# jatinagwal/kyverno

Measured on AMD Instinct MI355X. Metric: resource×rule evals/sec (background scan, PSS+best-practices) at 1/2/4/8 GPUs, higher is better.
Workload: dtype u32

## Files before the change

### __graft_entry__.py

```python
import os
import subprocess
import sys

ROOT = os.path.dirname(os.path.abspath(__file__))
if ROOT not in sys.path:
    sys.path.insert(0, ROOT)


def build():
    from kyverno_amd import build as B
    B.build()
    subprocess.run(["make", "-C", os.path.join(ROOT, "oracle"), "-j8"], check=True)
    import kyverno_amd
    from kyverno_amd import _lib
    _lib.lib()
    try:
        import concurrent.futures
        cache = os.path.join(ROOT, "kyverno_amd", "jitcache")
        jobs = [(wl, a) for wl in ("c3", "tests-c3", "c5", "c4", "c2") for a in (False, True)]
        try:
            sys.path.insert(0, os.path.join(ROOT, "tests"))
            import table_edge_cases
            jobs += [("tests-edges:%d" % i, False) for i in range(len(table_edge_cases.compiled_rulesets()))]
            import meta_keys_cases
            jobs += [("tests-metakeys%s:%d" % (off, i), a) for i in range(len(meta_keys_cases.compiled_rulesets()))
                     for off in ("", "-off") for a in (False, True)]
        except Exception as e:
            print("build: test rulesets not compiled ahead of time: %s" % e, file=sys.stderr)
        ctx = __import__("multiprocessing").get_context("spawn")
        with concurrent.futures.ProcessPoolExecutor(max_workers=min(len(jobs), os.cpu_count() or 1, 16), mp_context=ctx) as ex:
            list(ex.map(_aot_compile, jobs))
        t_start = {}
        ents = [f for f in os.listdir(cache) if f.endswith(".co")]
        for kind in ("walk", "acct"):
            newest = max((f for f in ents if f.startswith(kind + "-")), key=lambda f: os.path.getmtime(os.path.join(cache, f)))
            t_start[kind] = newest.split("-")[1]
        for f in os.listdir(cache):
            parts = f.split("-")
            if f.endswith(".co") and (len(parts) != 3 or t_start.get(parts[0]) != parts[1]):
                os.remove(os.path.join(cache, f))
    except Exception as e:
        print("build: ahead-of-time walk-kernel compile skipped: %s" % e, file=sys.stderr)
    try:
        _cache_bench_corpus()
    except Exception as e:
        print("build: bench corpus not prebuilt: %s" % e, file=sys.stderr)


def _cache_bench_corpus(total=10_000_000, need_free=14 << 30):
    import shutil
    import bench
    from kyverno_amd import synth
    if synth.corpus_is_cached(bench.CORPUS_CACHE, total, kind="mixed", seed=bench.SEED):
        return
    os.makedirs(bench.CORPUS_CACHE, exist_ok=True)
    free = shutil.disk_usage(bench.CORPUS_CACHE).free
    if free < need_free:
        raise RuntimeError("%.0f GB free under %s, %.0f GB wanted" % (free / 2**30, bench.CORPUS_CACHE, need_free / 2**30))
    synth.write_corpus_cache(bench.CORPUS_CACHE, total, kind="mixed", seed=bench.SEED)


def _aot_compile(job):
    if ROOT not in sys.path:
        sys.path.insert(0, ROOT)
    sys.path.insert(0, os.path.join(ROOT, "tests"))
    import bench
    import cases
    from kyverno_amd import engine as E
    wl, acct = job
    if wl.startswith("tests-edges:"):
        import table_edge_cases
        pols = table_edge_cases.compiled_rulesets()[int(wl.split(":")[1])]
    elif wl.startswith("tests-metakeys"):
        import meta_keys_cases
        pols = meta_keys_cases.compiled_rulesets()[int(wl.split(":")[1])]
        if wl.startswith("tests-metakeys-off:"):
            os.environ["KYV_META_KEYS"] = "0"
            try:
                return E.Ruleset(pols).jit_compile(accounting=acct)
            finally:
                del os.environ["KYV_META_KEYS"]
    else:
        pols = cases.best_practices() + cases.chart_restricted() if wl == "tests-c3" else bench.load_policies(wl)
    return E.Ruleset(pols).jit_compile(accounting=acct)


def smoke():
    sys.path.insert(0, os.path.join(ROOT, "tests"))
    import cases
    import parity_util as PU
    from kyverno_amd import synth

    docs, nsl = synth.mixed(300, seed=5, edge=True)
    pols = cases.best_practices()[:4] + cases.chart_restricted()[:6] + cases.quirk_policies()[-2:]
    st, res = PU.compare(pols, docs, nsl, backend="gpu")
    if st["nbad"]:
        raise AssertionError("GPU verdicts differ from the oracle: %r" % (st["bad"][:5],))
    if st["compared"] == 0:
        raise AssertionError("smoke compared no pairs")
    print("smoke ok: %d pairs, %d compared bit-exact vs oracle, kernel %.3f ms" % (st["pairs"], st["compared"],
                                                                                   res.kernel_ms))


if __name__ == "__main__":
    build() if (len(sys.argv) > 1 and sys.argv[1] == "build") else smoke()
```

### kyverno_amd/csrc/jit.cpp

```cpp
#include <dlfcn.h>
#include <sys/stat.h>
#include <unistd.h>
#include <hip/hip_runtime.h>
#include <hip/hiprtc.h>

#include <algorithm>
#include <chrono>
#include <cstdio>
#include <cstdlib>
#include <functional>
#include <map>
#include <mutex>
#include <utime.h>
#include <set>
#include <sstream>
#include <unordered_map>
#include <stdexcept>
#include <string>
#include <vector>

#include "kyv_host.h"

namespace kyv {

int pattern_depth(const Ruleset& rs, uint32_t pn, int guard);

bool jit_meta_keys_on() {
  const char* e = getenv("KYV_META_KEYS");
  return !e || atoi(e) != 0;
}

namespace {

struct Gen {
  const Ruleset& rs;
  std::ostringstream out;
  std::vector<uint8_t> emitted;
  std::vector<uint32_t> emitted_log;
  bool ok = true;
  const bool use_len = !getenv("KYV_JIT_LEN") || atoi(getenv("KYV_JIT_LEN")) != 0;
  const size_t batch_max = getenv("KYV_JIT_BATCH") ? (size_t)std::max(1, atoi(getenv("KYV_JIT_BATCH"))) : 1;
  const bool leaf_fast = !getenv("KYV_JIT_LEAF_FAST") || atoi(getenv("KYV_JIT_LEAF_FAST")) != 0;
  const bool meta_keys;
  static constexpr uint32_t MK_COL = 0x80000000u;
  struct WildSrc { int pc = -1; bool two = false; uint32_t cs = 0; };
  std::vector<int> slot_meta;
  std::vector<WildSrc> wild_src;
  WildSrc cur_src[MAX_SLOTS];
  int class_of(uint32_t pn) const {
    const PNode& P = rs.pnodes[pn];
    if (!meta_keys || !(P.flags & PF_META) || node_mbase[pn] == NONE || meta_pos[pn] < 0) return -1;
    const size_t s = (size_t)node_mbase[pn] + P.meta;
    return s < rs.meta_class_of.size() ? rs.meta_class_of[s] : -1;
  }

  std::vector<int> slot;
  std::vector<int> slot_alen;
  std::vector<int> slot_elen;
  std::vector<std::vector<uint32_t>> scope_of;
  std::vector<uint8_t> scoped;
  std::vector<uint32_t> node_mbase;
  std::vector<int8_t> meta_pos;

  explicit Gen(const Ruleset& r, int meta_keys_mode = -1)
      : rs(r), meta_keys(meta_keys_mode < 0 ? jit_meta_keys_on() : meta_keys_mode != 0), emitted(r.pnodes.size(), 0), slot_meta(r.pnodes.size(), -1), wild_src(r.pentries.size()),
        slot(r.pentries.size(), -1), slot_alen(r.pnodes.size(), -1),
        slot_elen(r.pentries.size(), -1), scope_of(r.pnodes.size()), scoped(r.pnodes.size(), 0),
        node_mbase(r.pnodes.size(), NONE), meta_pos(r.pnodes.size(), -1) {}

  void mark_paths(uint32_t pn, uint32_t mbase, uint32_t k0, uint32_t k1, uint32_t k2, uint32_t k3, int depth) {
    if (pn == NONE || pn >= rs.pnodes.size() || depth > 4) return;
    const PNode& P = rs.pnodes[pn];
    if (P.kind != P_MAP) return;
    node_mbase[pn] = mbase;
    const uint32_t S = SID_FIRST_FREE + K_SPEC, T = SID_FIRST_FREE + K_TEMPLATE, J = SID_FIRST_FREE + K_JOBTEMPLATE;
    if (depth == 0) meta_pos[pn] = 0;
    else if (depth == 2 && k0 == S && k1 == T) meta_pos[pn] = 1;
    else if (depth == 4 && k0 == S && k1 == J && k2 == S && k3 == T) meta_pos[pn] = 2;
    for (uint32_t e = 0; e < P.n; e++) {
      const PEntry& E = rs.pentries[P.first + e];
      if ((E.flags & EF_WILD) || E.child == NONE || E.handler == H_STAR || E.handler == H_NEGATION ||
          E.handler == H_EXISTENCE || E.handler == H_EXIST_BADPAT)
// ... 438 lines not shown
          out << "  if (" << c << " != NONE) return mkerr(EC_NONE, 0, " << ET << ");\n";
          break;
        case H_EXISTENCE: {
          uint32_t npat = rs.pool[E.child];
          out << "  if (" << c << " != NONE) {\n"
              << "    uint32_t cnt, eb, aa = NONE;\n";
          if (slot_elen[P.first + e] >= 0)
            out << "    if (" << t << " == N_ARR && (uint32_t)(pc[" << slot_elen[P.first + e] << "] >> 32) != NONE) {\n"
                << "      cnt = (uint32_t)pc[" << slot_elen[P.first + e] << "]; eb = (uint32_t)(pc[" << slot_elen[P.first + e]
                << "] >> 32);\n"
                << "    } else\n";
          out << "    { const Node a = gnode(w.R + " << c << ");\n"
              << "      if (node_type(a) != N_ARR) return mkerr(EC_NONE, 0, " << ET << ");\n"
              << "      cnt = a.b; eb = a.c; aa = a.a; }\n";
          for (uint32_t j = 0; j < npat; j++) {
            out << "    { bool hit = false;\n"
                << "      for (uint32_t i = 0; i < cnt; i++) {\n"
                << "        const uint32_t er = eb == NONE ? NONE : eb + i;\n"
                << "        " << preload(rs.pool[E.child + 1 + j], "pe", "er") << "\n"
                << "        uint32_t et = T_UNK, ea = 0u, ei = NONE;\n"
                << (rs.pe_self[P.first + e] != NONE ? "        ei = jdec(jself(w, " + u(rs.pe_self[P.first + e]) + ", er), &et, &ea);\n"
                                                      : std::string())
                << "        if (ei == NONE) { ei = aa + i; et = T_UNK; }\n"
                << "        Ret r = p" << rs.pool[E.child + 1 + j] << "(w, ei, et, ea, er, pe);\n"
                << "        if (w.ost) return r;\n"
                << "        if (!r.err) { hit = true; break; }\n"
                << "      }\n"
                << "      if (!hit) return mkerr(EC_NONE, 0, " << ET << "); }\n";
          }
          out << "  }\n";
          break;
        }
        default:
          out << "  {\n";
          call("");
          out << "  }\n";
      }
    }
    out << "  return ok_ret();\n";
  }
};

struct CondGen {
  const Ruleset& rs;
  std::ostringstream defs;
  std::ostringstream out;
  bool ok = true;
  uint32_t uid = 0;
  uint32_t nslots = 1;
  bool lds_used = false;
  uint32_t cur_etpos = NONE;
  std::unordered_map<uint64_t, std::string> progs;

  explicit CondGen(const Ruleset& r) : rs(r) {}
  static std::string u(uint32_t x) { return std::to_string(x) + "u"; }
  std::string fresh(const char* p) { return std::string(p) + std::to_string(uid++); }

  uint32_t tchild(uint32_t t, uint32_t key) const {
    if (t == NONE) return NONE;
    for (auto& kv : rs.trie[t].kids) if (kv.first == key) return kv.second;
    return NONE;
  }
  uint32_t tstar(uint32_t t) const { return t == NONE ? NONE : rs.trie[t].star; }
  uint32_t tcol(uint32_t t) const { return t == NONE ? NONE : rs.trie[t].col; }
  uint32_t tlen(uint32_t t) const { return t == NONE || rs.trie[t].star == NONE ? NONE : rs.trie[t].lencol; }

  struct V {
    std::string i, t, a, row;
    uint32_t tpos;
    bool key;
  };
  V decl(const std::string& i, const std::string& t, const std::string& a, const std::string& row, uint32_t tpos,
         bool key) {
    V x{fresh("vi"), fresh("vt"), fresh("va"), fresh("vr"), tpos, key};
    out << "  uint32_t " << x.i << " = " << i << ", " << x.t << " = " << t << ", " << x.a << " = " << a << ", " << x.row
        << " = " << row << ";\n";
    return x;
  }
  V field(const V& x, uint32_t key) {
    if (x.key) return decl("NONE", "T_UNK", "0u", "NONE", NONE, false);
    const uint32_t ct = tchild(x.tpos, key), col = tcol(ct);
    V y{fresh("vi"), fresh("vt"), fresh("va"), fresh("vr"), col == NONE ? NONE : ct, false};
    out << "  uint32_t " << y.i << ", " << y.t << ", " << y.a << ";\n"
        << "  jc_field(v, R, " << x.i << ", " << x.row << ", " << (col == NONE ? "NONE" : u(col)) << ", " << u(key) << ", &"
        << y.i << ", &" << y.t << ", &" << y.a << ");\n"
        << "  const uint32_t " << y.row << " = " << (col == NONE ? std::string("NONE") : x.row) << ";\n";
    return y;
  }
  bool unroll = false;
  V open_elems(const V& x, const std::string& notarr_then, const char* on_arr = "") {
    const std::string cnt = fresh("cn"), aa = fresh("aa"), eb = fresh("eb"), j = fresh("j");
    const uint32_t st = tstar(x.tpos);
    out << "  { uint32_t " << cnt << " = 0u, " << aa << " = 0u, " << eb << " = NONE;\n"
        << "  if (" << (x.key ? "false" : "jc_arr(v, R, " + x.i + ", " + x.t + ", " + x.a + ", " + x.row + ", " +
                                              (tlen(x.tpos) == NONE ? std::string("NONE") : u(tlen(x.tpos))) + ", &" + cnt +
                                              ", &" + aa + ", &" + eb + ")")
        << ") {\n" << on_arr << (unroll ? "  KYV_JC_UNROLL\n" : "")
        << "  for (uint32_t " << j << " = 0; " << j << " < " << cnt << "; " << j << "++) {\n";
    V e{fresh("vi"), fresh("vt"), fresh("va"), fresh("vr"), st, false};
    out << "  uint32_t " << e.i << ", " << e.t << ", " << e.a << ", " << e.row << ";\n"
        << "  jc_elem(v, R, " << aa << ", " << (st == NONE ? std::string("NONE") : eb) << ", " << j << ", "
        << (tcol(st) == NONE ? std::string("NONE") : u(tcol(st))) << ", &" << e.i << ", &" << e.t << ", &" << e.a << ", &"
        << e.row << ");\n";
    pending_else.push_back(notarr_then);
    return e;
  }
  std::vector<std::string> pending_else;
  void close_loop() {
    out << "  }\n  }";
    std::string e = pending_else.back();
    pending_else.pop_back();
    if (!e.empty()) out << " else {\n" << e << "  }";
    out << "\n  }\n";
  }

  const uint32_t* P = nullptr;
  uint32_t PN = 0, PEND = 0;
  bool streaming = false;
  std::string sacc;
  void jend(const V& x, bool list, bool proj) {
    if (!list) {
      out << "  *cur = " << (x.key ? "(" + x.i + " | JMES_KEYBIT)" : x.i) << ";\n";
      return;
    }
    if (streaming) {
      std::string sx;
      if (x.key) sx = "(gtk(R + " + x.i + ") >> 4)";
      else sx = "jc_sprint(R, " + x.i + ", " + x.t + ", " + x.a + ")";
      const std::string body = "{ const uint32_t es = " + sx + ";\n    if (++*ln > JCAP) return JS_FB;\n    " + sacc + " }";
      if (x.key) out << "  " << body << "\n";
      else if (proj) out << "  if (" << x.i << " != NONE) " << body << "\n";
      else out << "  " << body << "\n";
      return;
    }
    const std::string e = x.key ? "jc_keyent(R, " + x.i + ")" : "jc_ent(" + x.i + ", " + x.t + ", " + x.a + ")";
    if (x.key) out << "  if (!jc_push(L, ln, " << e << ")) return JS_FB;\n";
    else if (proj) out << "  if (" << x.i << " != NONE) { if (!jc_push(L, ln, " << e << ")) return JS_FB; }\n";
    else out << "  if (!jc_push(L, ln, " << x.i << " == NONE ? NONE : " << e << ")) return JS_FB;\n";
  }
  void jgen(uint32_t pos, const V& x, bool list, bool proj, int guard) {
    if (!ok || guard > 64) { ok = false; return; }
    if (pos >= PEND) { jend(x, list, proj); return; }
    const uint32_t op = P[pos];
    switch (op) {
      case JO_FIELD: {
        out << "  {\n";
        V y = field(x, P[pos + 1]);
        jgen(pos + 2, y, list, proj, guard + 1);
        out << "  }\n";
        return;
      }
      case JO_MULTI: {
        if (list) { ok = false; return; }
        const uint32_t m = P[pos + 1];
        out << "  if (" << x.i << " == NONE) {\n";
        jgen(pos + 2 + m, x, false, proj, guard + 1);
        out << "  } else {\n  *lst = true;\n";
        for (uint32_t o = 0; o < m; o++) {
          out << "  {\n";
          V y = field(x, P[pos + 2 + o]);
          jgen(pos + 2 + m, y, true, proj, guard + 1);
          out << "  }\n";
        }
        out << "  }\n";
        return;
      }
      case JO_FLAT: {
        if (!list) {
          std::ostringstream save;
          save.swap(out);
          V nul{"NONE", "T_UNK", "0u", "NONE", NONE, false};
          jgen(pos + 1, nul, false, false, guard + 1);
          std::string notarr = out.str();
          out.swap(save);
          V e = open_elems(x, notarr, "  *lst = true;\n");
          jgen(pos + 1, e, true, true, guard + 1);
          close_loop();
          return;
        }
        out << "  if (" << (proj && !x.key ? x.i + " != NONE" : std::string("true")) << ") {\n";
        std::ostringstream save;
        save.swap(out);
        V pass{x.i, x.t, x.a, "NONE", NONE, x.key};
        jgen(pos + 1, pass, true, true, guard + 1);
        std::string notarr = out.str();
        out.swap(save);
        V e = open_elems(x, notarr);
        jgen(pos + 1, e, true, true, guard + 1);
        close_loop();
        out << "  }\n";
        return;
      }
      case JO_KEYS: {
        if (list) { ok = false; return; }
// ... 326 lines not shown
         << "(const View& v, const Node* R, uint32_t r, uint32_t ei, uint32_t et, uint32_t ea, uint32_t erow, uint32_t* L) {\n"
         << "  (void)ei; (void)et; (void)ea; (void)erow;\n"
         << b << "}\n";
    progs[key] = name;
    return name;
  }

  const ForeachEntry* FE = nullptr;
  void elem_body(const V& e) {
    out << "  do {\n";
    if (FE->scope == 2) out << "  if (jc_type(R, " << e.i << ", " << e.t << ") != N_MAP) return ST_ERROR | ST_MARK_SCOPE;\n";
    out << "  bool err = false;\n";
    const std::string args = "(v, R, r, " + e.i + ", " + e.t + ", " + e.a + ", " + e.row + ", L)";
    if (FE->pre != NONE) {
      const std::string f = prog_fn(FE->pre, e.tpos);
      out << "  { const int c = " << f << args << ";\n"
          << "    if (c == CR_FB) return ST_FALLBACK;\n    if (c == CR_PANIC) return ST_PANIC;\n"
          << "    if (c == CR_FALSE) break;\n    err = c == CP_ERROR; }\n";
    }
    const std::string f = prog_fn(FE->deny, e.tpos);
    out << "  if (!err) { const int c = " << f << args << ";\n"
        << "    if (c == CR_FB) return ST_FALLBACK;\n    if (c == CR_PANIC) return ST_PANIC;\n"
        << "    if (c == CR_TRUE) return ST_FAIL;\n    if (c != CP_ERROR) { count++; break; } }\n"
        << "  pend = true;\n  } while (0);\n";
  }
  void fend(const V& x, bool list, bool proj) {
    if (x.key) { ok = false; return; }
    if (list) {
      if (proj) {
        out << "  if (" << x.i << " != NONE) {\n  pend = false;\n";
        elem_body(x);
        out << "  }\n";
      } else {
        out << "  pend = false;\n  if (" << x.i << " != NONE) {\n";
        elem_body(x);
        out << "  }\n";
      }
      return;
    }
    std::ostringstream save;
    save.swap(out);
    out << "  pend = false;\n  if (" << (x.i == "NONE" ? std::string("false") : x.i + " != NONE && jc_type(R, " + x.i + ", " + x.t + ") != N_NULL")
        << ") {\n";
    elem_body(x);
    out << "  }\n";
    const std::string single = out.str();
    out.swap(save);
    V e = open_elems(x, single);
    out << "  pend = false;\n  if (" << e.i << " != NONE) {\n";
    elem_body(e);
    out << "  }\n";
    close_loop();
  }
  void fgen(uint32_t pos, const V& x, bool list, bool proj, int guard) {
    if (!ok || guard > 64) { ok = false; return; }
    if (pos >= PEND) { fend(x, list, proj); return; }
    const uint32_t op = P[pos];
    switch (op) {
      case JO_FIELD: {
        out << "  {\n";
        V y = field(x, P[pos + 1]);
        fgen(pos + 2, y, list, proj, guard + 1);
        out << "  }\n";
        return;
      }
      case JO_MULTI: {
        if (list) { ok = false; return; }
        const uint32_t m = P[pos + 1];
        out << "  if (" << x.i << " == NONE) {\n";
        fgen(pos + 2 + m, x, false, proj, guard + 1);
        out << "  } else {\n";
        for (uint32_t o = 0; o < m; o++) {
          out << "  {\n";
          V y = field(x, P[pos + 2 + o]);
          fgen(pos + 2 + m, y, true, proj, guard + 1);
          out << "  }\n";
        }
        out << "  }\n";
        return;
      }
      case JO_FLAT: {
        std::ostringstream save;
        save.swap(out);
        if (!list) {
          V nul{"NONE", "T_UNK", "0u", "NONE", NONE, false};
          fgen(pos + 1, nul, false, false, guard + 1);
        } else {
          V pass{x.i, x.t, x.a, "NONE", NONE, x.key};
          fgen(pos + 1, pass, true, true, guard + 1);
        }
        const std::string notarr = out.str();
        out.swap(save);
        if (list) out << "  if (" << (proj ? x.i + " != NONE" : std::string("true")) << ") {\n";
        V e = open_elems(x, notarr);
        fgen(pos + 1, e, true, true, guard + 1);
        close_loop();
        if (list) out << "  }\n";
        return;
      }
      default: ok = false; return;
    }
  }
  void foreach_entry(const ForeachEntry& fe) {
    FE = &fe;
    out << "  { uint32_t count = 0u; bool pend = false; bool skip = false; (void)skip;\n";
    const CondOperand& o = fe.list;
    const uint32_t* p = o.kind == OK_JMES ? rs.pool.data() + o.a : nullptr;
    const bool chain = o.kind == OK_PATH || (p && (p[0] & JF_PURE));
// ... 104 lines not shown
  const uint32_t nany = p.nany == NONE ? 0u : p.nany;
  for (uint32_t i = 0; i < nany; i++)
    if (heavy_jmes(rs, rs.conds[p.any0 + i].key) || heavy_jmes(rs, rs.conds[p.any0 + i].value)) return true;
  for (uint32_t i = 0; i < p.nall; i++)
    if (heavy_jmes(rs, rs.conds[p.all0 + i].key) || heavy_jmes(rs, rs.conds[p.all0 + i].value)) return true;
  return false;
}

std::string self_dir() {
  Dl_info info;
  if (dladdr((void*)&self_dir, &info) && info.dli_fname) {
    std::string p = info.dli_fname;
    size_t s = p.rfind('/');
    return s == std::string::npos ? std::string(".") : p.substr(0, s);
  }
  return ".";
}

}

constexpr uint32_t kFusedGW = 8;
bool jit_rule_fused(const Ruleset& rs, uint32_t k) {
  static const bool on = !getenv("KYV_FUSED") || atoi(getenv("KYV_FUSED")) != 0;
  if (!on || k >= rs.rules.size() || rs.rules.size() > 32u * kFusedGW) return false;
  const RuleDesc& rd = rs.rules[k];
  return (rd.kind == RK_PATTERN || rd.kind == RK_ANYPATTERN) && (rd.flags & RD_GATE_EXACT);
}

bool jit_shape_eligible(const Ruleset& rs, uint32_t k) {
  static const bool on = !getenv("KYV_SHAPES") || atoi(getenv("KYV_SHAPES")) != 0;
  if (!on || k >= rs.rules.size()) return false;
  const RuleDesc& rd = rs.rules[k];
  return rd.kind == RK_PATTERN && rd.pre == NONE && !(rd.flags & RD_GATE_EXACT) && !jit_rule_fused(rs, k);
}

static std::string meta_signature(const Ruleset& rs, const RuleDesc& rd) {
  std::string o;
  if (!rd.uses_meta) return o;
  auto pool = [&](uint32_t at, uint32_t n) {
    for (uint32_t i = 0; i < 2 * n && at + i < rs.pool.size(); i++) o += std::to_string(rs.pool[at + i]) + ",";
  };
  for (uint32_t i = 0; i < rd.nmeta && rd.meta_sites + i < rs.metas.size(); i++) {
    const MetaSite& m = rs.metas[rd.meta_sites + i];
    o += "[" + std::to_string(m.has_labels) + "," + std::to_string(m.has_ann) + "," + std::to_string(m.nwild_l) + ":";
    pool(m.wild_l, m.nwild_l);
    o += std::to_string(m.nwild_a) + ":";
    pool(m.wild_a, m.nwild_a);
    o += std::to_string(m.slot_l) + "," + std::to_string(m.slot_a) + "]";
  }
  return o;
}

std::string jit_source(const Ruleset& rs, std::vector<uint8_t>* jit_rules, std::vector<uint8_t>* jit_cond,
                       std::vector<uint16_t>* jit_shape, int meta_keys) {
  Gen g(rs, meta_keys);
  jit_rules->assign(rs.rules.size(), 0);
  if (jit_shape) jit_shape->assign(rs.rules.size(), 0);
  if (jit_cond) jit_cond->assign(rs.rules.size(), 0);
  const size_t cap = getenv("KYV_JIT_MAX_RULES") ? (size_t)atol(getenv("KYV_JIT_MAX_RULES")) : 1024;
  CondGen cg(rs);
  std::vector<uint32_t> crules;
  const bool cond_on = !getenv("KYV_JIT_COND") || atoi(getenv("KYV_JIT_COND")) != 0;
  for (size_t k = 0; k < rs.rules.size() && cond_on && crules.size() < cap; k++) {
    const RuleDesc& rd = rs.rules[k];
    if (rd.kind != RK_DENY && rd.kind != RK_FOREACH) continue;
    if (rd.kind == RK_DENY && !prog_has_jmes(rs, rd.pre) && !prog_has_jmes(rs, rd.root)) continue;
    const std::string mark = cg.defs.str();
    const auto progs = cg.progs;
    cg.ok = true;
    cg.rule_fn((uint32_t)k);
    if (!cg.ok) {
      cg.defs.str("");
      cg.defs.clear();
      cg.defs << mark;
      cg.progs = progs;
      continue;
    }
    crules.push_back((uint32_t)k);
  }
  std::vector<std::pair<uint32_t, std::vector<uint32_t>>> rule_roots;
  std::ostringstream body;
  std::unordered_map<std::string, uint32_t> shapes;
  std::unordered_map<uint32_t, uint32_t> rep_of;
  auto canon = [](const std::string& t) {
    std::unordered_map<std::string, size_t> ids;
    std::string o;
    o.reserve(t.size());
    for (size_t i = 0; i < t.size();) {
      if (t[i] == 'p' && (i == 0 || !(isalnum((unsigned char)t[i - 1]) || t[i - 1] == '_')) && i + 1 < t.size() &&
          isdigit((unsigned char)t[i + 1])) {
        size_t j = i + 1;
        while (j < t.size() && isdigit((unsigned char)t[j])) j++;
        if (j < t.size() && t[j] == '(') {
          auto it = ids.emplace(t.substr(i, j - i), ids.size()).first;
          o += "p#" + std::to_string(it->second);
          i = j;
          continue;
        }
      }
      o += t[i++];
    }
    return o;
  };
  size_t nshapes = 0;
  const bool only_cond = getenv("KYV_JIT_ONLY_COND") && atoi(getenv("KYV_JIT_ONLY_COND")) != 0;
  for (size_t k = 0; k < rs.rules.size() && !only_cond; k++) {
    const RuleDesc& rd = rs.rules[k];
    if (rd.kind != RK_PATTERN && rd.kind != RK_ANYPATTERN) continue;
    std::vector<uint32_t> rr;
    if (rd.kind == RK_PATTERN) rr.push_back(rd.root);
    else for (uint32_t a = 0; a < rd.nalts; a++) rr.push_back(rs.pool[rd.root + a]);
    bool ok = true;
    for (uint32_t r : rr) if (pattern_depth(rs, r, 0) > MAX_DEPTH) ok = false;
// ... 644 lines not shown
```

### kyverno_amd/csrc/kyv_engine.hip

```cpp
#define KYV_SEL_INLINE 1
#include <hip/hip_runtime.h>

#include <algorithm>
#include <array>
#include <map>
#include <chrono>
#include <cmath>
#include <functional>
#include <cstdlib>
#include <mutex>
#include <set>
#include <cstdio>
#include <cstring>
#include <stdexcept>
#include <string>
#include <thread>
#include <vector>

#include "kyv_acct.h"
#include "kyv_host.h"
#define KYV_NO_KERNELS 1
#include "kyv_kernels.h"

namespace kyv {
// ... 765 lines not shown
    }
    out[(size_t)s * words + w] = bits;
  }
}

int pattern_depth(const Ruleset& rs, uint32_t pn, int guard) {
  if (pn == NONE || guard > MAX_DEPTH) return MAX_DEPTH + 1;
  const PNode& P = rs.pnodes[pn];
  int d = 0;
  switch (P.kind) {
    case P_MAP:
      for (uint32_t e = 0; e < P.n; e++) {
        const PEntry& E = rs.pentries[P.first + e];
        if (E.handler == H_STAR || E.handler == H_NEGATION || E.child == NONE) continue;
        if (E.handler == H_EXISTENCE || E.handler == H_EXIST_BADPAT) {
          uint32_t npat = rs.pool[E.child];
          for (uint32_t j = 0; j < npat; j++) d = std::max(d, 1 + pattern_depth(rs, rs.pool[E.child + 1 + j], guard + 2));
        } else {
          d = std::max(d, pattern_depth(rs, E.child, guard + 1));
        }
      }
      return 1 + d;
    case P_ARR_MAPS: return 1 + pattern_depth(rs, P.first, guard + 1);
    case P_ARR_POS:
      for (uint32_t i = 0; i < P.n; i++) d = std::max(d, pattern_depth(rs, rs.pool[P.first + i], guard + 1));
      return 1 + d;
    default: return 0;
  }
}

static int ruleset_depth(const Ruleset& rs) {
  int d = 1;
  for (auto& rd : rs.rules) {
    if (rd.kind == RK_PATTERN) d = std::max(d, pattern_depth(rs, rd.root, 0));
    else if (rd.kind == RK_ANYPATTERN)
      for (uint32_t a = 0; a < rd.nalts; a++) d = std::max(d, pattern_depth(rs, rs.pool[rd.root + a], 0));
  }
  return std::min(d, (int)MAX_DEPTH);
}


static std::mutex g_jit_mu;
static void mrs_clear_shapes(Ruleset& rs) {
  std::fill(rs.jit_shape.begin(), rs.jit_shape.end(), (uint16_t)0);
  rs.jit_nshapes = 0;
}
static bool ensure_jit(Ruleset& rs, DevRuleset* dr) {
  if (dr->jloaded) return true;
  std::lock_guard<std::mutex> lk(g_jit_mu);
  if (!rs.jit_tried) {
    rs.jit_tried = true;
    try {
      rs.jit_meta_keys = jit_meta_keys_on() && !rs.meta_classes.empty();
      std::string src = jit_source(rs, &rs.jit_rules, &rs.jit_cond, &rs.jit_shape, rs.jit_meta_keys ? 1 : 0);
      rs.jit_nshapes = 0;
      for (auto x : rs.jit_shape) rs.jit_nshapes = std::max<uint32_t>(rs.jit_nshapes, x);
      bool any = false;
      for (auto x : rs.jit_rules) any |= x != 0;
      for (auto x : rs.jit_cond) any |= x != 0;
      if (any) rs.jit_code = jit_compile(src, &rs.jit_compile_s);
    } catch (std::exception& e) {
      rs.jit_error = e.what();
      rs.jit_code.clear();
      fprintf(stderr, "[kyvgpu] runtime-compiled walk kernel unavailable, using the interpreted one: %s\n", e.what());
    }
  }
  if (rs.jit_code.empty()) return false;
  HIP_OK(hipModuleLoadData(&dr->jmod, rs.jit_code.data()));
  uint32_t ng = 0;
  for (auto x : rs.jit_rules) ng = std::max<uint32_t>(ng, x);
  dr->jfns.resize(ng);
  dr->ffns.assign(ng, nullptr);
  for (uint32_t g = 0; g < ng; g++) {
    HIP_OK(hipModuleGetFunction(&dr->jfns[g], dr->jmod, ("kyv_jit_walk_" + std::to_string(g)).c_str()));
    if (hipModuleGetFunction(&dr->ffns[g], dr->jmod, ("kyv_jit_fused_" + std::to_string(g)).c_str()) != hipSuccess)
      dr->ffns[g] = nullptr;
    dr->fparts.resize(ng);
    for (int p = 1; dr->ffns[g]; p++) {
      hipFunction_t f = nullptr;
      if (hipModuleGetFunction(&f, dr->jmod, ("kyv_jit_fused_" + std::to_string(g) + "p" + std::to_string(p)).c_str()) != hipSuccess)
        break;
      dr->fparts[g].push_back(f);
    }
    dr->fmfns.resize(ng, nullptr);
    if (hipModuleGetFunction(&dr->fmfns[g], dr->jmod, ("kyv_jit_fusedm_" + std::to_string(g)).c_str()) != hipSuccess)
      dr->fmfns[g] = nullptr;
  }
  (void)hipGetLastError();
  dr->jshapes = nullptr;
  if (rs.jit_nshapes && hipModuleGetFunction(&dr->jshapes, dr->jmod, "kyv_jit_shapes") != hipSuccess) {
    dr->jshapes = nullptr;
    mrs_clear_shapes(rs);
  }
  (void)hipGetLastError();
  dr->jconds.assign(rs.rules.size(), nullptr);
  dr->jc_group.assign(rs.rules.size(), -1);
  dr->jcg.clear();
  dr->jcg_members.clear();
  {
    std::vector<uint32_t> crules;
    for (size_t k = 0; k < rs.jit_cond.size(); k++) if (rs.jit_cond[k] == 1) crules.push_back((uint32_t)k);
    for (auto& grp : jit_cond_groups(rs, crules)) {
      hipFunction_t f = nullptr;
      if (hipModuleGetFunction(&f, dr->jmod, ("kyv_jit_condg_" + std::to_string(grp[0])).c_str()) != hipSuccess) continue;
      for (uint32_t k : grp) dr->jc_group[k] = (int32_t)dr->jcg.size();
      dr->jcg.push_back(f);
      dr->jcg_members.push_back(grp);
    }
    (void)hipGetLastError();
  }
  for (size_t k = 0; k < rs.jit_cond.size(); k++)
    if (rs.jit_cond[k] == 1 && dr->jc_group[k] < 0)
      HIP_OK(hipModuleGetFunction(&dr->jconds[k], dr->jmod, ("kyv_jit_cond_" + std::to_string(k)).c_str()));
  dr->jloaded = true;
  return true;
}

static bool ensure_jit_acct(Ruleset& rs, DevRuleset* dr) {
  if (dr->aloaded) return true;
  if (!ensure_jit(rs, dr)) return false;
  std::lock_guard<std::mutex> lk(g_jit_mu);
  if (rs.jit_code_acct.empty()) {
    std::vector<uint8_t> jr, jc;
    rs.jit_code_acct = jit_compile(jit_source(rs, &jr, &jc, nullptr, rs.jit_meta_keys ? 1 : 0), nullptr, true);
  }
  HIP_OK(hipModuleLoadData(&dr->amod, rs.jit_code_acct.data()));
  dr->afns.resize(dr->jfns.size());
  dr->affns.assign(dr->jfns.size(), nullptr);
  for (size_t g = 0; g < dr->jfns.size(); g++) {
    HIP_OK(hipModuleGetFunction(&dr->afns[g], dr->amod, ("kyv_jit_walk_" + std::to_string(g)).c_str()));
    if (dr->ffns[g]) HIP_OK(hipModuleGetFunction(&dr->affns[g], dr->amod, ("kyv_jit_fused_" + std::to_string(g)).c_str()));
    dr->afparts.resize(dr->jfns.size());
    dr->afparts[g].assign(g < dr->fparts.size() ? dr->fparts[g].size() : 0, nullptr);
    for (size_t p = 0; p < dr->afparts[g].size(); p++)
      HIP_OK(hipModuleGetFunction(&dr->afparts[g][p], dr->amod,
                                  ("kyv_jit_fused_" + std::to_string(g) + "p" + std::to_string(p + 1)).c_str()));
    dr->afmfns.resize(dr->jfns.size(), nullptr);
    if (g < dr->fmfns.size() && dr->fmfns[g])
      HIP_OK(hipModuleGetFunction(&dr->afmfns[g], dr->amod, ("kyv_jit_fusedm_" + std::to_string(g)).c_str()));
  }
  dr->aconds.assign(dr->jconds.size(), nullptr);
  for (size_t k = 0; k < dr->jconds.size(); k++)
    if (dr->jconds[k]) HIP_OK(hipModuleGetFunction(&dr->aconds[k], dr->amod, ("kyv_jit_cond_" + std::to_string(k)).c_str()));
  dr->ajshapes = nullptr;
  if (dr->jshapes) HIP_OK(hipModuleGetFunction(&dr->ajshapes, dr->amod, "kyv_jit_shapes"));
  dr->ajcg.assign(dr->jcg.size(), nullptr);
  for (size_t g = 0; g < dr->jcg.size(); g++)
    HIP_OK(hipModuleGetFunction(&dr->ajcg[g], dr->amod, ("kyv_jit_condg_" + std::to_string(dr->jcg_members[g][0])).c_str()));
  hipDeviceptr_t p = nullptr;
  size_t bytes = 0;
  HIP_OK(hipModuleGetGlobal(&p, &bytes, dr->amod, "kyv_acct_bytes"));
  dr->acnt = (unsigned long long*)p;
  dr->aloaded = true;
  return true;
}

static size_t rule_slice_bytes(const RuleDesc& rd) {
  const size_t alts = rd.kind == RK_PATTERN ? 1 : rd.kind == RK_ANYPATTERN ? std::min<uint32_t>(rd.nalts, MAX_ALTS) : 0;
  return sizeof(uint2) + 2 * alts * sizeof(FailRec) + 1;
}

static size_t slice_budget() {
  if (const char* e = getenv("KYV_SLICE_MB")) return (size_t)std::max(1, atoi(e)) << 20;
  size_t fr = 0, tot = 0;
  if (hipMemGetInfo(&fr, &tot) != hipSuccess || fr == 0) fr = (size_t)64 << 30;
  return std::min<size_t>(fr / 2, (size_t)128 << 30);
}

static void build_mrec(const Ruleset& rs, uint32_t q, const std::vector<uint32_t>& gidx, bool masks_on, bool on, MRec& R) {
  memset(&R, 0, sizeof R);
  const RuleDesc& rd = rs.rules[q];
  R.k = q;
  R.kind = rd.kind;
  R.flags = rd.flags;
  bool fast = on && rd.match.mode != MM_NONE && rd.exc == NONE && rd.match.nfilters + rd.exclude.nfilters <= MREC_F;
  bool uses = false;
  auto pat = [&](uint32_t sid) -> uint32_t {
// ... 1799 lines not shown
```

### kyverno_amd/csrc/kyv_host.h

```cpp
#pragma once
#include <cstdint>
#include <functional>
#include <memory>
#include <string>
#include <unordered_map>
#include <vector>

#include "kyv_layout.h"
#include "pjson.h"

namespace kyv {

template <class T>
struct NoInitAlloc : std::allocator<T> {
  template <class U> struct rebind { using other = NoInitAlloc<U>; };
  NoInitAlloc() = default;
  template <class U> NoInitAlloc(const NoInitAlloc<U>&) noexcept {}
  template <class U> void construct(U* p) noexcept { ::new ((void*)p) U; }
  template <class U, class... A> void construct(U* p, A&&... a) { ::new ((void*)p) U(std::forward<A>(a)...); }
};
template <class T> using bulk_vector = std::vector<T, NoInitAlloc<T>>;

struct Dict {
  std::vector<std::string> strs;
// ... 50 lines not shown
  std::vector<uint16_t> next;
  std::vector<uint8_t> accept;
  bool end_anchor = false;
};
bool rx_compile(const std::string& re, RxDfa* out, std::string* why);
int rx_match(const RxDfa& d, const uint8_t* s, size_t n);

struct Ruleset {
  Dict dict;
  std::vector<RuleDesc> rules;
  std::vector<RuleMeta> meta;
  std::vector<PolicyMeta> policies;
  std::vector<Filter> filters;
  std::vector<KindDesc> kinds;
  std::vector<SelDesc> sels;
  std::vector<SelReq> reqs;
  std::vector<PNode> pnodes;
  std::vector<PEntry> pentries;
  std::vector<Leaf> leaves;
  std::vector<Atom> atoms;
  std::vector<MetaSite> metas;
  std::vector<PssDesc> pss;
  std::vector<uint32_t> pool;
  std::vector<Node> cnodes;
  std::vector<Cond> conds;
  std::vector<CondProg> cprogs;
  std::vector<CondText> cond_text;
  std::vector<std::string> templates;
  std::unordered_map<std::string, uint32_t> template_ids;
  struct TrieNode {
    uint32_t col = NONE;
    uint32_t rowspace = 0;
    uint32_t star = NONE;
    uint32_t lencol = NONE;
    std::vector<std::pair<uint32_t, uint32_t>> kids;
  };
  std::vector<TrieNode> trie;
  std::vector<uint32_t> gpats;
  std::vector<std::vector<uint32_t>> gsets;
  std::vector<uint32_t> cond_set;
  std::vector<std::string> rx_src;
  std::vector<RxDfa> rxs;
  bool uses_upper = false;
  uint32_t ncols = 0, nrowspaces = 1;
  std::vector<uint32_t> col_rowspace;
  std::vector<uint32_t> pn_self;
  std::vector<uint32_t> pe_self;
  std::vector<uint32_t> pn_len;
  std::vector<uint32_t> pe_len;
  std::vector<uint32_t> fact_spaces;
  std::vector<MetaClass> meta_classes;
  std::vector<int8_t> meta_class_of;
  bool jit_meta_keys = false;
  bool jit_tried = false;
  std::vector<uint8_t> jit_rules;
  std::vector<uint8_t> jit_cond;
  std::vector<uint16_t> jit_shape;
  uint32_t jit_nshapes = 0;
  std::vector<char> jit_code;
  std::vector<char> jit_code_acct;
  std::string jit_error;
  double jit_compile_s = 0;
  std::vector<void*> dev;
  ~Ruleset();
};

struct TypedDecoder {
  enum Target { POD = 0, DEPLOYMENT = 1, CRONJOB = 2 };
  explicit TypedDecoder(const std::function<uint32_t(const std::string&)>& find_sid);
  enum Outcome { DEC_OK = 0, DEC_ERR = 1, DEC_FOLD = 2 };
  int decode(const Node* R, const std::vector<std::string>& strs, int target) const;
  std::unordered_map<uint32_t, uint32_t> name_of_sid;
};

struct Batch {
  const Ruleset* rs = nullptr;
  Dict dict;
  bulk_vector<Node> nodes;
  bulk_vector<ResHeader> hdr;
  bulk_vector<HotHdr> hot;
  std::vector<FloatAux> faux;
  std::vector<uint32_t> str_off, str_len, str_flags;
  std::vector<uint32_t> str_upper, str_rx;
  std::vector<int64_t> str_dur, str_qty;
  std::vector<double> str_f64;
  std::vector<uint8_t> heap;
  std::vector<uint32_t> nsl_off, nsl_kv;
  std::vector<std::string> nsl_names;
  std::vector<uint32_t> order;
  std::vector<uint32_t> inv;
  std::vector<uint64_t> shape_key;
  std::shared_ptr<const std::vector<uint32_t>> inv_shared;
  std::vector<uint32_t> gate;
  uint32_t gate_words = 0, nclass = 0;
  bulk_vector<uint64_t> colv;
  std::vector<uint32_t> col_off, rs_rows;
  std::vector<WaveFacts> facts;
  std::vector<void*> dev;
  ~Batch();
};

struct FailPath {
  uint32_t res, rule, alt;
  uint32_t tmpl;
  uint16_t idx[MAX_IDX];
  uint32_t key[2];
};

struct SlicePlan { uint32_t k0 = 0, k1 = 0, fused = 0, chunk = 0, cond = 0; };
struct EvalPlan {
  uint32_t gmask_patterns = 0, cond_sets = 0, gmask_words = 0, unmasked = 0;
  uint32_t onemask = 0;
  uint32_t tail_used[5] = {0, 0, 0, 0, 0};
  uint32_t tail_cand[5] = {0, 0, 0, 0, 0};
  uint32_t fast = 0, fasteval = 0, generic = 0;
};
void plan_ruleset(const Ruleset& rs, EvalPlan* p);

struct Results {
  uint32_t nres = 0, nrules = 0;
  EvalPlan plan;
  std::vector<SlicePlan> slices;
  std::vector<uint8_t> status;
  std::vector<uint32_t> pss_fails;
  std::vector<FailRec> fails;
  int64_t counts[NSTATUS] = {0};
  std::vector<int64_t> rule_counts;
  double kernel_ms = 0, h2d_ms = 0, d2h_ms = 0;
  double gmask_ms = 0;
  double meta_keys_ms = 0;
  double phase_ms[5] = {0, 0, 0, 0, 0};
  uint64_t alg_bytes = 0;
  uint64_t alg_bytes_phase[5] = {0, 0, 0, 0, 0};
  uint64_t alg_bytes_class[3] = {0, 0, 0};
  int jit_used = 0;
};

Ruleset* compile_ruleset(const char* json, size_t len, std::string* err, const char* exceptions = nullptr,
                         size_t ex_len = 0, bool background = false);
Batch* build_batch(const Ruleset* rs, const char* json, size_t len, const char* nsl_json, size_t nsl_len, int threads,
                   std::string* err);
void derive_strings(Batch& b, size_t from, int threads);
void build_path_trie(Ruleset& rs);
void assign_wave_facts(Ruleset& rs);
void assign_meta_classes(Ruleset& rs);
bool jit_meta_keys_on();
std::vector<MetaKeyRow> meta_key_rows_host(const Ruleset& rs, const Batch& b);
std::vector<MetaKeyRow> meta_key_rows_device(const Batch& b, int device);
size_t meta_key_plane_bytes(const Batch& b);
uint32_t wave_maps_mask();
void assign_glob_masks(Ruleset& rs);
void assign_cond_sets(Ruleset& rs);
std::string jit_source(const Ruleset& rs, std::vector<uint8_t>* jit_rules, std::vector<uint8_t>* jit_cond = nullptr,
                       std::vector<uint16_t>* jit_shape = nullptr, int meta_keys = -1);
bool jit_shape_eligible(const Ruleset& rs, uint32_t k);
constexpr uint32_t JIT_MAX_SHAPES = 64;
std::vector<char> jit_compile(const std::string& src, double* seconds, bool acct = false);
bool jit_rule_fused(const Ruleset& rs, uint32_t k);
std::vector<std::vector<uint32_t>> jit_cond_groups(const Ruleset& rs, const std::vector<uint32_t>& crules);
struct KindGate {
  bool any = false;
  std::vector<uint32_t> kinds;
};
KindGate rule_gate(const Ruleset& rs, const RuleDesc& rd);
enum JitMode { JIT_AUTO = 0, JIT_OFF = 1, JIT_ON = 2 };
constexpr size_t JIT_AUTO_MIN_RESOURCES = 65536;
void resolve_path_columns(Batch& b, int threads);
constexpr uint32_t SHAPE_KEY_BITS = 3, SHAPE_KEY_MAX_NODES = 64 / SHAPE_KEY_BITS;
std::vector<uint32_t> shape_key_nodes(const Ruleset& rs);
std::string format_path(const Ruleset& rs, const Batch& b, uint32_t tmpl, const uint16_t* idx, const uint32_t* key);

}
```

### kyverno_amd/csrc/kyv_jcond.h

```cpp
#pragma once
#include "kyv_wave.h"
#include "kyv_cond.h"
#include "kyv_pss.h"

namespace kyv {

constexpr uint32_t JCAP = 16;

__device__ __forceinline__ uint64_t jc_col(const View& v, uint32_t col, uint32_t row) {
  if (row == NONE) return COL_NONE;
  KYV_ACCT_ADDK(2u, 0, 8);
  const uint32_t off = sld32(v.col_off + col);
  return gcol(v.colv, off, row);
}
__device__ __forceinline__ kyv_u32x4 jc_meta(const View& v, uint32_t cls, uint32_t row) {
  if (row == NONE) return kyv_u32x4{0u, NONE, NONE, NONE};
  KYV_ACCT_ADD(0, 16);
  return *(const KYV_AS_GLOBAL kyv_u32x4*)(v.meta_rows + ((size_t)cls * v.nres + row));
}
__device__ __forceinline__ uint32_t jc_dec(uint64_t x, uint32_t* t, uint32_t* a) {
  const uint32_t lo = (uint32_t)x;
  *a = (uint32_t)(x >> 32);
  if (lo == NONE) { *t = T_UNK; *a = 0; return NONE; }
  *t = lo >> COL_TYPE_SHIFT;
  return lo & COL_INDEX_MASK;
}
__device__ __forceinline__ uint32_t jc_type(const Node* R, uint32_t i, uint32_t t) {
  if (i == NONE) return N_NULL;
  return t != T_UNK ? t : (gtk(R + i) & 0xFu);
}
__device__ __forceinline__ void jc_field(const View& v, const Node* R, uint32_t i, uint32_t row, uint32_t col, uint32_t key,
                                         uint32_t* oi, uint32_t* ot, uint32_t* oa) {
  *ot = T_UNK;
  *oa = 0;
  if (col != NONE && row != NONE) {
    uint32_t x = jc_dec(jc_col(v, col, row), ot, oa);
    if (x != NONE && *ot == N_NULL) { x = NONE; *ot = T_UNK; *oa = 0; }
    *oi = x;
    return;
  }
  if (i == NONE) { *oi = NONE; return; }
  const Node m = gnode(R + i);
  if (node_type(m) != N_MAP) { *oi = NONE; return; }
  const uint32_t x = wmap_find(R, m.a, m.b, key);
  if (x == NONE) { *oi = NONE; return; }
  const Node n = gnode(R + x);
  if (node_type(n) == N_NULL) { *oi = NONE; return; }
  *oi = x;
  *ot = node_type(n);
  *oa = n.a;
}
__device__ __forceinline__ bool jc_arr(const View& v, const Node* R, uint32_t i, uint32_t t, uint32_t a, uint32_t row,
                                       uint32_t lencol, uint32_t* cnt, uint32_t* aa, uint32_t* eb) {
  if (i == NONE) return false;
  if (t != T_UNK && t != N_ARR) return false;
  if (t == N_ARR && lencol != NONE && row != NONE) {
    const uint64_t x = jc_col(v, lencol, row);
    if ((uint32_t)x != NONE) { *cnt = (uint32_t)x; *eb = (uint32_t)(x >> 32); *aa = a; return true; }
  }
  const Node n = gnode(R + i);
  if (node_type(n) != N_ARR) return false;
  *cnt = n.b;
  *aa = n.a;
  *eb = n.c;
  return true;
}
__device__ __forceinline__ void jc_elem(const View& v, const Node* R, uint32_t aa, uint32_t eb, uint32_t j, uint32_t self,
                                        uint32_t* oi, uint32_t* ot, uint32_t* oa, uint32_t* orow) {
  *oi = aa + j;
  *ot = T_UNK;
  *oa = 0;
  *orow = eb == NONE ? NONE : eb + j;
  if (self != NONE && *orow != NONE) {
    uint32_t t, a;
    if (jc_dec(jc_col(v, self, *orow), &t, &a) != NONE) { *ot = t; *oa = a; }
  }
  if (jc_type(R, *oi, *ot) == N_NULL) { *oi = NONE; *ot = T_UNK; *oa = 0; }
}
__device__ __forceinline__ uint32_t jc_ent(uint32_t i, uint32_t t, uint32_t a) {
  return (t == N_STR && a < JMES_SIDBIT) ? (a | JMES_SIDBIT) : i;
}
__device__ __forceinline__ uint32_t jc_keyent(const Node* R, uint32_t idx) {
  const uint32_t k = gtk(R + idx) >> 4;
  return k < JMES_SIDBIT ? (k | JMES_SIDBIT) : (idx | JMES_KEYBIT);
}
__device__ __forceinline__ bool jc_push(uint32_t* L, uint32_t* n, uint32_t e) {
  if (*n >= JCAP) return false;
  L[(size_t)*n << 6] = e;
  (*n)++;
  return true;
}
__device__ __forceinline__ bool jc_false1(const Node* R, uint32_t cur) {
  if (cur == NONE) return true;
  if (cur & JMES_KEYBIT) return node_key(gnode(R + (cur & ~JMES_KEYBIT))) == SID_EMPTY;
  const Node n = gnode(R + cur);
  switch (node_type(n)) {
    case N_NULL: case N_FALSE: return true;
    case N_STR: return n.a == SID_EMPTY;
    case N_ARR: case N_MAP: return n.b == 0;
    default: return false;
  }
}
__device__ __forceinline__ uint32_t jc_sprint(const Node* R, uint32_t i, uint32_t t, uint32_t a) {
// ... 41 lines not shown
```

Baseline: 146.8 billion.

## Collapse chained field lookups into a single preloaded column read in JIT conditions

The condition JIT generator now defers consecutive field accesses along a path whose final trie node has a precomputed column. It emits one column lookup for the whole chain, and falls back to walking the tree node by node only when no row is available. The aim is to replace several dependent global-memory node reads per path with a single column read. It adds an environment switch, a code-generation path that keeps lazy chain state, and extra ahead-of-time test compile jobs. Correctness depends on the column encoding matching the result of the full chain walk.

Measured after the change: 152.0 billion, median of 6. +3.6%, better.

```diff
diff --git a/__graft_entry__.py b/__graft_entry__.py
--- a/__graft_entry__.py
+++ b/__graft_entry__.py
@@ -24,6 +24,9 @@
             jobs += [("tests-edges:%d" % i, False) for i in range(len(table_edge_cases.compiled_rulesets()))]
             import meta_keys_cases
             jobs += [("tests-metakeys%s:%d" % (off, i), a) for i in range(len(meta_keys_cases.compiled_rulesets()))
+                     for off in ("", "-off") for a in (False, True)]
+            import cond_preload_cases
+            jobs += [("tests-condpre%s:%d" % (off, i), a) for i in range(len(cond_preload_cases.compiled_rulesets()))
                      for off in ("", "-off") for a in (False, True)]
         except Exception as e:
             print("build: test rulesets not compiled ahead of time: %s" % e, file=sys.stderr)
@@ -80,6 +83,15 @@
                 return E.Ruleset(pols).jit_compile(accounting=acct)
             finally:
                 del os.environ["KYV_META_KEYS"]
+    elif wl.startswith("tests-condpre"):
+        import cond_preload_cases
+        pols = cond_preload_cases.compiled_rulesets()[int(wl.split(":")[1])]
+        if wl.startswith("tests-condpre-off:"):
+            os.environ["KYV_JC_PRELOAD"] = "0"
+            try:
+                return E.Ruleset(pols).jit_compile(accounting=acct)
+            finally:
+                del os.environ["KYV_JC_PRELOAD"]
     else:
         pols = cases.best_practices() + cases.chart_restricted() if wl == "tests-c3" else bench.load_policies(wl)
     return E.Ruleset(pols).jit_compile(accounting=acct)
diff --git a/kyverno_amd/csrc/jit.cpp b/kyverno_amd/csrc/jit.cpp
--- a/kyverno_amd/csrc/jit.cpp
+++ b/kyverno_amd/csrc/jit.cpp
@@ -28,6 +28,11 @@
 bool jit_meta_keys_on() {
   const char* e = getenv("KYV_META_KEYS");
   return !e || atoi(e) != 0;
+}
+
+int jit_jc_chains_mode() {
+  const char* e = getenv("KYV_JC_PRELOAD");
+  return e ? (atoi(e) != 0) : jit_meta_keys_on() ? 1 : 0;
 }
 
 namespace {
@@ -572,7 +577,7 @@
   uint32_t cur_etpos = NONE;
   std::unordered_map<uint64_t, std::string> progs;
 
-  explicit CondGen(const Ruleset& r) : rs(r) {}
+  CondGen(const Ruleset& r, int mode) : rs(r), chains(mode < 0 ? jit_jc_chains_mode() != 0 : mode != 0) {}
   static std::string u(uint32_t x) { return std::to_string(x) + "u"; }
   std::string fresh(const char* p) { return std::string(p) + std::to_string(uid++); }
 
@@ -589,7 +594,21 @@
     std::string i, t, a, row;
     uint32_t tpos;
     bool key;
+    std::vector<uint32_t> lz;
   };
+  const bool chains;
+  V force(const V& x) {
+    if (x.lz.empty()) return x;
+    V y{fresh("vi"), fresh("vt"), fresh("va"), x.row, x.tpos, false, {}};
+    out << "  uint32_t " << y.i << ", " << y.t << ", " << y.a << ";\n"
+        << "  if (" << x.row << " != NONE) jc_field_e(jc_col(v, " << u(tcol(x.tpos)) << ", " << x.row << "), &" << y.i << ", &"
+        << y.t << ", &" << y.a << ");\n"
+        << "  else {\n    " << y.i << " = " << x.i << ";\n";
+    for (uint32_t key : x.lz)
+      out << "    jc_field(v, R, " << y.i << ", NONE, NONE, " << u(key) << ", &" << y.i << ", &" << y.t << ", &" << y.a << ");\n";
+    out << "  }\n";
+    return y;
+  }
   V decl(const std::string& i, const std::string& t, const std::string& a, const std::string& row, uint32_t tpos,
          bool key) {
     V x{fresh("vi"), fresh("vt"), fresh("va"), fresh("vr"), tpos, key};
@@ -597,8 +616,15 @@
         << " = " << row << ";\n";
     return x;
   }
-  V field(const V& x, uint32_t key) {
-    if (x.key) return decl("NONE", "T_UNK", "0u", "NONE", NONE, false);
+  V field(const V& x0, uint32_t key) {
+    if (x0.key) return decl("NONE", "T_UNK", "0u", "NONE", NONE, false);
+    if (chains && tcol(tchild(x0.tpos, key)) != NONE) {
+      V y = x0;
+      y.tpos = tchild(x0.tpos, key);
+      y.lz.push_back(key);
+      return y;
+    }
+    const V x = force(x0);
     const uint32_t ct = tchild(x.tpos, key), col = tcol(ct);
     V y{fresh("vi"), fresh("vt"), fresh("va"), fresh("vr"), col == NONE ? NONE : ct, false};
     out << "  uint32_t " << y.i << ", " << y.t << ", " << y.a << ";\n"
@@ -658,8 +684,9 @@
     else if (proj) out << "  if (" << x.i << " != NONE) { if (!jc_push(L, ln, " << e << ")) return JS_FB; }\n";
     else out << "  if (!jc_push(L, ln, " << x.i << " == NONE ? NONE : " << e << ")) return JS_FB;\n";
   }
-  void jgen(uint32_t pos, const V& x, bool list, bool proj, int guard) {
+  void jgen(uint32_t pos, const V& x0, bool list, bool proj, int guard) {
     if (!ok || guard > 64) { ok = false; return; }
+    const V x = pos < PEND && P[pos] == JO_FIELD ? x0 : force(x0);
     if (pos >= PEND) { jend(x, list, proj); return; }
     const uint32_t op = P[pos];
     switch (op) {
@@ -1092,8 +1119,9 @@
     out << "  }\n";
     close_loop();
   }
-  void fgen(uint32_t pos, const V& x, bool list, bool proj, int guard) {
+  void fgen(uint32_t pos, const V& x0, bool list, bool proj, int guard) {
     if (!ok || guard > 64) { ok = false; return; }
+    const V x = pos < PEND && P[pos] == JO_FIELD ? x0 : force(x0);
     if (pos >= PEND) { fend(x, list, proj); return; }
     const uint32_t op = P[pos];
     switch (op) {
@@ -1304,13 +1332,13 @@
 }
 
 std::string jit_source(const Ruleset& rs, std::vector<uint8_t>* jit_rules, std::vector<uint8_t>* jit_cond,
-                       std::vector<uint16_t>* jit_shape, int meta_keys) {
+                       std::vector<uint16_t>* jit_shape, int meta_keys, int jc_chains) {
   Gen g(rs, meta_keys);
   jit_rules->assign(rs.rules.size(), 0);
   if (jit_shape) jit_shape->assign(rs.rules.size(), 0);
   if (jit_cond) jit_cond->assign(rs.rules.size(), 0);
   const size_t cap = getenv("KYV_JIT_MAX_RULES") ? (size_t)atol(getenv("KYV_JIT_MAX_RULES")) : 1024;
-  CondGen cg(rs);
+  CondGen cg(rs, jc_chains);
   std::vector<uint32_t> crules;
   const bool cond_on = !getenv("KYV_JIT_COND") || atoi(getenv("KYV_JIT_COND")) != 0;
   for (size_t k = 0; k < rs.rules.size() && cond_on && crules.size() < cap; k++) {
diff --git a/kyverno_amd/csrc/kyv_engine.hip b/kyverno_amd/csrc/kyv_engine.hip
--- a/kyverno_amd/csrc/kyv_engine.hip
+++ b/kyverno_amd/csrc/kyv_engine.hip
@@ -841,7 +841,8 @@
     rs.jit_tried = true;
     try {
       rs.jit_meta_keys = jit_meta_keys_on() && !rs.meta_classes.empty();
-      std::string src = jit_source(rs, &rs.jit_rules, &rs.jit_cond, &rs.jit_shape, rs.jit_meta_keys ? 1 : 0);
+      rs.jit_jc_chains = jit_jc_chains_mode();
+      std::string src = jit_source(rs, &rs.jit_rules, &rs.jit_cond, &rs.jit_shape, rs.jit_meta_keys ? 1 : 0, rs.jit_jc_chains);
       rs.jit_nshapes = 0;
       for (auto x : rs.jit_shape) rs.jit_nshapes = std::max<uint32_t>(rs.jit_nshapes, x);
       bool any = false;
@@ -911,7 +912,7 @@
   std::lock_guard<std::mutex> lk(g_jit_mu);
   if (rs.jit_code_acct.empty()) {
     std::vector<uint8_t> jr, jc;
-    rs.jit_code_acct = jit_compile(jit_source(rs, &jr, &jc, nullptr, rs.jit_meta_keys ? 1 : 0), nullptr, true);
+    rs.jit_code_acct = jit_compile(jit_source(rs, &jr, &jc, nullptr, rs.jit_meta_keys ? 1 : 0, rs.jit_jc_chains), nullptr, true);
   }
   HIP_OK(hipModuleLoadData(&dr->amod, rs.jit_code_acct.data()));
   dr->afns.resize(dr->jfns.size());
diff --git a/kyverno_amd/csrc/kyv_host.h b/kyverno_amd/csrc/kyv_host.h
--- a/kyverno_amd/csrc/kyv_host.h
+++ b/kyverno_amd/csrc/kyv_host.h
@@ -126,6 +126,7 @@
   std::vector<MetaClass> meta_classes;
   std::vector<int8_t> meta_class_of;
   bool jit_meta_keys = false;
+  int jit_jc_chains = 0;
   bool jit_tried = false;
   std::vector<uint8_t> jit_rules;
   std::vector<uint8_t> jit_cond;
@@ -225,8 +226,9 @@
 uint32_t wave_maps_mask();
 void assign_glob_masks(Ruleset& rs);
 void assign_cond_sets(Ruleset& rs);
+int jit_jc_chains_mode();
 std::string jit_source(const Ruleset& rs, std::vector<uint8_t>* jit_rules, std::vector<uint8_t>* jit_cond = nullptr,
-                       std::vector<uint16_t>* jit_shape = nullptr, int meta_keys = -1);
+                       std::vector<uint16_t>* jit_shape = nullptr, int meta_keys = -1, int jc_chains = -1);
 bool jit_shape_eligible(const Ruleset& rs, uint32_t k);
 constexpr uint32_t JIT_MAX_SHAPES = 64;
 std::vector<char> jit_compile(const std::string& src, double* seconds, bool acct = false);
diff --git a/kyverno_amd/csrc/kyv_jcond.h b/kyverno_amd/csrc/kyv_jcond.h
--- a/kyverno_amd/csrc/kyv_jcond.h
+++ b/kyverno_amd/csrc/kyv_jcond.h
@@ -49,6 +49,11 @@
   *oi = x;
   *ot = node_type(n);
   *oa = n.a;
+}
+__device__ __forceinline__ void jc_field_e(uint64_t e, uint32_t* oi, uint32_t* ot, uint32_t* oa) {
+  uint32_t x = jc_dec(e, ot, oa);
+  if (x != NONE && *ot == N_NULL) { x = NONE; *ot = T_UNK; *oa = 0; }
+  *oi = x;
 }
 __device__ __forceinline__ bool jc_arr(const View& v, const Node* R, uint32_t i, uint32_t t, uint32_t a, uint32_t row,
                                        uint32_t lencol, uint32_t* cnt, uint32_t* aa, uint32_t* eb) {
```
